# dafyddstephenson/ucla-roms

Hardware: AMD Instinct MI355X
Metric: grid-cell-updates/sec (higher is better)
Workload: dtype f64; 1 GPU; C3: basin 1024x1024x100, NONLIN+SPLIT EOS, T+S, LMD KPP/BKPP/RIMIX/NONLOCAL, dt=300s, ndtfast=60 (nfast=82); NT=2, nfast=82, parallelism=domain decomposition 1x1, halo_transport=none (single rank), fast_exchange_interval=1, exchange_order=none (single rank), s2d_window=True, comm_bootstrap=none (single rank)

## Files before the change

include/roms_gpu.h:

```cpp
#ifndef ROMS_GPU_H
#define ROMS_GPU_H

#ifdef __cplusplus
extern "C" {
#endif

#define ROMS_GPU_ABI_VERSION 23
#define ROMS_MAX_FAST 288

typedef struct roms_dims {
  int Lm, Mm, N, NT;
  int LLm, MMm;
  int np_xi, np_eta, inode, jnode;
  int iSW_corn, jSW_corn;
  int ew_periodic, ns_periodic;
  int west_exchng, east_exchng, south_exchng, north_exchng;
} roms_dims;

#define ROMS_LMD_MIXING   1
#define ROMS_LMD_KPP      2
#define ROMS_LMD_BKPP     4
#define ROMS_LMD_RIMIX    8
#define ROMS_LMD_CONVEC   16
#define ROMS_LMD_NONLOCAL 32
#define ROMS_LMD_ALL      63
#define ROMS_LMD_ICELAND  47
#define ROMS_LMD_DDMIX    64

typedef struct roms_cfg {
  int nonlin_eos;
  int salinity;
  int lmd_mixing;
  int uv_vis2, ts_dif2;
  double dt;
  int ndtfast, nfast;
  double weight[2][ROMS_MAX_FAST];
  double g, rho0, rdrg, rdrg2, Zob, gamma2;
  double Akv_bak, Akt_bak[2];
  double Tcoef, T0, Scoef, S0;
  double theta_s, theta_b, hc;
  int obc;
  double ubind;
  int curvgrid;
  int uv_adv, uv_cor;
  int pot_tides;
  int bulk_frc;
  int adv_isoneutral;
} roms_cfg;

typedef struct roms_tlev {
  int iic, ntstart, forw_start, iif, nfast, kstp, knew, nstp, nrhs, nnew;
} roms_tlev;

enum roms_field {
  ROMS_ALL = -1,
  ROMS_h = 0, ROMS_hinv, ROMS_f, ROMS_fomn, ROMS_pm, ROMS_pn, ROMS_dm_r, ROMS_dn_r, ROMS_dm_u, ROMS_dn_u,
  ROMS_dm_v, ROMS_dn_v, ROMS_dm_p, ROMS_dn_p, ROMS_pmon_u, ROMS_pnom_v, ROMS_rmask, ROMS_pmask, ROMS_umask,
  ROMS_vmask,
  ROMS_Cs_w, ROMS_Cs_r,
  ROMS_zeta, ROMS_ubar, ROMS_vbar, ROMS_u, ROMS_v, ROMS_t, ROMS_FlxU, ROMS_FlxV, ROMS_We, ROMS_Wi,
// ... 37 lines not shown
int roms_gpu_pre_step3d(const roms_tlev *t);
int roms_gpu_set_huv1(const roms_tlev *t);
int roms_gpu_step3d_uv1(const roms_tlev *t);
int roms_gpu_visc3d(const roms_tlev *t);
int roms_gpu_step2d(const roms_tlev *t);
int roms_gpu_step3d_uv2(const roms_tlev *t);
int roms_gpu_step3d_t(const roms_tlev *t);
int roms_gpu_t3dmix(const roms_tlev *t);
int roms_gpu_swr_frac(const roms_tlev *t);
int roms_gpu_set_pipe_frc(int npip, const int *pipe_idx, const double *pipe_flx, const double *pipe_prf,
                          const double *pipe_trc);
int roms_gpu_set_river_frc(int nriv, const double *riv_uflx, const double *riv_vflx, const double *riv_vol,
                           const double *riv_trc);
int roms_gpu_bulk_flux(const roms_tlev *t);
int roms_gpu_set_ub_tune(const double *ub_west, const double *ub_east, const double *ub_south, const double *ub_north);
int roms_gpu_set_depth(const roms_tlev *t);

int roms_gpu_step(roms_tlev *t);
int roms_gpu_init_sequence(roms_tlev *t);

enum roms_case_id { ROMS_CASE_FILAMENT = 0, ROMS_CASE_BASIN = 1, ROMS_CASE_PIPES = 2, ROMS_CASE_RIVERS = 3 };
typedef struct roms_case {
  int case_id, LLm, MMm, N, NT;
  int salinity, nonlin_eos, lmd_mixing;
  double dt; int ndtfast;
  double sizex, sizey;
  int surf_flux;
  int obc;
  double v_sponge;
  int island;
  int curvgrid;
  int uv_adv, uv_cor;
  int bulk_frc;
  int adv_isoneutral;
} roms_case;
int roms_gpu_init_case(const roms_case *c, int device, roms_tlev *t);
int roms_gpu_init_case_comm(const roms_case *c, int np_xi, int np_eta, void *comm, int device, roms_tlev *t);

int roms_gpu_comm_unique_id(void *id128);
int roms_gpu_comm_create(const void *id128, int nranks, int rank, int device, void **comm);
int roms_gpu_comm_create_local(int group, int nranks, int rank, void **comm);
typedef int (*roms_host_allgather_fn)(void *ctx, const void *send, long nbytes, void *recv);
int roms_gpu_comm_create_host(int nranks, int rank, int device, roms_host_allgather_fn allgather, void *ctx,
                              void **comm);
int roms_gpu_comm_destroy(void *comm);
int roms_gpu_halo_transport(void);
int roms_gpu_halo_exchanges(long *per_step, int *fast_interval);
int roms_gpu_halo_overlap(void);
int roms_gpu_s2d_window(void);
#define ROMS_COLPATH_SEG 1
#define ROMS_COLPATH_GLOBAL 2
int roms_gpu_column_path(void);
int roms_gpu_kpp_lean(void);
int roms_gpu_vgrid(void);
int roms_gpu_vgrid2(void);
int roms_gpu_vgrid_check(long out[3]);
int roms_gpu_tracer_pair(long launches[2]);
int roms_gpu_tracer_hstg(long launches[3]);
int roms_gpu_horizontal_path(int out[8]);
int roms_gpu_selftest_zero_fill(long n, int chunks, long *bad);
int roms_gpu_halo_plan(int Lm, int Mm, int np_xi, int np_eta, int inode, int jnode, int ew_periodic,
                       int ns_periodic, int peer[8], long count[8], int strip[4]);
long roms_gpu_halo_map(int Lm, int Mm, int np_xi, int np_eta, int inode, int jnode, int ew_periodic,
                       int ns_periodic, int dir, int unpack, int *i, int *j, long cap);
long roms_gpu_halo_map_wide(int Lm, int Mm, int np_xi, int np_eta, int inode, int jnode, int ew_periodic,
                            int ns_periodic, int width, int dir, int unpack, int *i, int *j, long cap);

#define ROMS_FRC_SURFACE 1
#define ROMS_FRC_BRY     2
int roms_gpu_frc_record(int field_id, int slot, double rec_time, const double *data);
int roms_gpu_frc_interp(double modtime, int kinds);
int roms_gpu_frc_clock(double start_time, int on);
int roms_gpu_set_tide_data(int ntides, const double *ftide, const double *pot_re, const double *pot_im,
                           const double *ztide_re, const double *ztide_im, const double *utide_re,
                           const double *utide_im, const double *vtide_re, const double *vtide_im);
int roms_gpu_set_tides(double time);

#define ROMS_WRT_Z    1
#define ROMS_WRT_UB   2
#define ROMS_WRT_VB   4
#define ROMS_WRT_U    8
#define ROMS_WRT_V    16
#define ROMS_WRT_T    32
#define ROMS_WRT_R    64
#define ROMS_WRT_O    128
#define ROMS_WRT_AKV  256
#define ROMS_WRT_AKT  512
#define ROMS_WRT_AKS  1024
#define ROMS_WRT_HBLS 2048
#define ROMS_WRT_HBBL 4096
#define ROMS_WRT_DEFAULT 63
int roms_gpu_wrt_rst(const char *path, int rec, int total_rec, double time, const roms_tlev *t);
int roms_gpu_wrt_his(const char *path, int rec, int total_rec, double time, const roms_tlev *t, int wrt_mask);
int roms_gpu_io_wait(void);
int roms_gpu_io_tracer_name(int itrc, const char *name, const char *units, const char *long_name);
int roms_gpu_get_init(const char *path, int req_rec, int tindx, roms_tlev *t, double *start_time);

int roms_gpu_diag(const roms_tlev *t, double norms[4]);
int roms_gpu_set_weights(int ndtfast, double weight[2][ROMS_MAX_FAST]);
int roms_gpu_time_steps(roms_tlev *t, int n, double *ms);
enum roms_routine {
  ROMS_R_RHO_EOS = 0, ROMS_R_SET_HUV, ROMS_R_OMEGA, ROMS_R_PRSGRD, ROMS_R_PRE_STEP3D, ROMS_R_SET_HUV1,
  ROMS_R_STEP3D_UV1, ROMS_R_VISC3D, ROMS_R_STEP2D, ROMS_R_STEP3D_UV2, ROMS_R_STEP3D_T, ROMS_R_T3DMIX,
  ROMS_R_LMD_VMIX,
  ROMS_R_K_S2D_FB,
  ROMS_R_K_PRE_UV_SEG,
// ... 15 lines not shown
```

ucla-roms_amd/csrc/k_lmd.hip:

```cpp
#include <cmath>
#include <type_traits>

#include "k_common.h"

namespace roms {
namespace {

constexpr double kRicr = 0.15, kEpssfc = 0.1, kC_Ek = 258.;
constexpr double kZeta_m = -0.2, kA_m = 1.257, kC_m = 8.360, kZeta_s = -1.0, kA_s = -28.86, kC_s = 98.96;
constexpr double kEPS = 1.E-20;
constexpr double kRi0 = 0.7, kNu0m = 1.e-2, kNu0s = 1.e-2, kNuwm = 1.0e-4, kNuws = 0.1e-4, kNu0c = 0.1, kLturb = 10.;
constexpr double kPi = 3.14159265358979323;

__device__ __forceinline__ void ddmix(double t0, double t1, double s0, double s1, double zwk, double& kt,
                                      double& ks) {
  const double A0 = +0.665157E-01, A1 = +0.170907E-01, A2 = -0.203814E-03, A3 = +0.298357E-05,
               A4 = -0.255019E-07, B0 = +0.378110E-02, B1 = -0.846960E-04, C0 = -0.678662E-05,
               D0 = +0.380374E-04, D1 = -0.933746E-06, D2 = +0.791325E-08, E0 = -0.164759E-06,
               F0 = -0.251520E-11, G0 = +0.512857E-12, H0 = -0.302285E-13, Smean = 35.0;
  const double lmd_nu = 1.5e-6, lmd_Rrho0 = 1.9, lmd_nuf = 10.0e-4, lmd_fdd = 0.7, lmd_tdd1 = 0.909,
               lmd_tdd2 = 4.6, lmd_tdd3 = 0.54, lmd_sdd1 = 0.15, lmd_sdd2 = 1.85, lmd_sdd3 = 0.85, eps = 1.E-14;
  const double Tt = 0.5 * (t0 + t1);
  const double Ts = 0.5 * (s0 + s1) - Smean;
  const double Tp = -zwk;
// ... 97 lines not shown
  for (int dj = 0; dj < 2; dj++)
#pragma unroll
    for (int di = 0; di < 3; di++) FE1[dj][di] = (w[dj + 1][di] - w[dj][di]) * m.vm[dj][di];
  const double FEj = FE1[0][1] + cff * (FX[1][1] + FX[0][0] - FX[1][0] - FX[0][1]);
  const double FEjp = FE1[1][1] + cff * (FX[2][1] + FX[1][0] - FX[2][0] - FX[1][1]);
  const double FXi = FX[1][0] + cff * (FE1[1][1] + FE1[0][0] - FE1[0][1] - FE1[1][0]);
  const double FXip = FX[1][1] + cff * (FE1[1][2] + FE1[0][1] - FE1[0][2] - FE1[1][1]);
  return w[1][1] + cff1 * (FXip - FXi + FEjp - FEj);
}

__device__ __forceinline__ void load3x3(const Bounds& b, const EdgeClamp& ec, const double* a, int i, int j,
                                        double (&w)[3][3]) {
#pragma unroll
  for (int dj = 0; dj < 3; dj++)
#pragma unroll
    for (int di = 0; di < 3; di++) w[dj][di] = a[ec.at(b, i - 1 + di, j - 1 + dj)];
}

__global__ void __launch_bounds__(256) k_swr_frac(Dev d, Range R) {
  ROMS_IJ_OR_RETURN(R)
  const Bounds& b = d.b;
  const long ij = IJ(b, i, j), n2 = b.n2;
  const int N = b.N;
  const double mu1 = 0.35, mu2 = 23.0, r1 = 0.58;
  const double attn1 = -1. / mu1, attn2 = -1. / mu2;
  double swdk1 = r1, swdk2 = 1. - swdk1;
  double* __restrict__ sw = d.f.swr_frac + ij;
  const double* __restrict__ Hz = d.f.Hz + ij;
  sw[(long)N * n2] = 1.;
  for (int k = N; k >= 1; k--) {
    const double hz = Hz[(long)(k - 1) * n2];
    const double xi1 = attn1 * hz;
    if (xi1 > -20.) swdk1 = swdk1 * exp(xi1);
    else swdk1 = 0.;
    const double xi2 = attn2 * hz;
    if (xi2 > -20.) swdk2 = swdk2 * exp(xi2);
    else swdk2 = 0.;
    sw[(long)(k - 1) * n2] = swdk1 + swdk2;
  }
}

#ifndef ROMS_KBLS_G
#define ROMS_KBLS_G 16
#endif
constexpr int kKblsG = ROMS_KBLS_G;
#ifndef ROMS_KPP_PFD
#define ROMS_KPP_PFD 1
#endif
constexpr int kKppPfd = ROMS_KPP_PFD;

#ifndef ROMS_KPP_EXT_WAVES
#define ROMS_KPP_EXT_WAVES 3
#endif
template <class C, bool KEEP = false, bool VG = false>
__global__ void __launch_bounds__(64, ROMS_KPP_EXT_WAVES) k_kpp_ext(Dev d, Range E, int tind, int nstp, KppConst kc) {
  ROMS_IJC_OR_RETURN(E)
  const Bounds& b = d.b;
  const Fields& F = d.f;
  const Params& P = d.p;
  const int N = b.N;
  const long n2 = b.n2, ij = IJ(b, i, j), sj = b.nx2;
  const double g = P.g, vonKar = P.vonKar, Ri_inv = 1. / kRicr;
  const C FCc = ColMake<C>::at(d, 0, 0, ij);
  const BufF64 FCg(d.f.colscr);
  constexpr bool kGlb = std::is_same<C, ColGlb>::value;
  static_assert(!KEEP || std::is_same<C, ColLds>::value, "KEEP: the LDS slot");
  const int keep = KEEP ? (P.kpp_fckeep < N ? P.kpp_fckeep : N) : N;
  auto fc_set = [&](int k, double v) {
    if constexpr (kGlb) FCg.st(v, (unsigned)ij * 8u, (unsigned)k * (unsigned)n2 * 8u);
    else if (!KEEP || k <= keep) FCc[k] = v;
  };
  auto fc_get = [&](int k) {
    if constexpr (kGlb) return FCg.ld((unsigned)ij * 8u, (unsigned)k * (unsigned)n2 * 8u);
    else return FCc[k];
  };
  double alpha, beta;
  const double Tt = F.t[ij + (long)(N - 1) * n2 + (long)(nstp - 1) * b.n3];
  if (P.nonlin_eos) {
    const double r01 = 6.793952E-2, r02 = -9.095290E-3, r03 = +1.001685E-4, r04 = -1.120083E-6,
                 r05 = +6.536332E-9, r10 = +0.824493, r11 = -4.08990E-3, r12 = +7.64380E-5,
                 r13 = -8.24670E-7, r14 = +5.38750E-9, rS0 = -5.72466E-3, rS1 = +1.02270E-4,
                 rS2 = -1.65460E-6, r20 = +4.8314E-4;
    const double cff = 1. / P.rho0;
    if (P.salinity) {
      const double Ts = F.t[ij + (long)(N - 1) * n2 + (long)(nstp - 1) * b.n3 + 3 * b.n3], sqrtTs = sqrt(dmax(0., Ts));
      alpha = -cff * (r01 + Tt * (2. * r02 + Tt * (3. * r03 + Tt * (4. * r04 + Tt * 5. * r05))) +
                      Ts * (r11 + Tt * (2. * r12 + Tt * (3. * r13 + Tt * 4. * r14)) + sqrtTs * (rS1 + Tt * 2. * rS2)));
      beta = cff * (r10 + Tt * (r11 + Tt * (r12 + Tt * (r13 + Tt * r14))) + 1.5 * (rS0 + Tt * (rS1 + Tt * rS2)) * sqrtTs +
                    2. * r20 * Ts);
    } else {
      alpha = -cff * (r01 + Tt * (2. * r02 + Tt * (3. * r03 + Tt * (4. * r04 + Tt * 5. * r05))));
      beta = 0.;
    }
  } else {
    alpha = fabs(P.Tcoef);
    beta = P.salinity ? fabs(P.Scoef) : 0.;
  }
  const double sr = F.srflx[ij];
  const double Bo = P.salinity ? g * (alpha * (F.stflx[ij] - sr) - beta * F.stflx[ij + n2]) : g * (alpha * (F.stflx[ij] - sr));
  const double Bosol = g * alpha * sr;
  double ustar;
  if (P.bulk_frc) {
    const double sr_ = F.sustr_r[ij], sv_ = F.svstr_r[ij];
    ustar = sqrt(sqrt(sr_ * sr_ + sv_ * sv_));
  } else {
    const double su0 = F.sustr[ij], su1 = F.sustr[ij + 1], sv0 = F.svstr[ij], sv1 = F.svstr[ij + sj];
    ustar = sqrt(sqrt(0.333333333333 * (su0 * su0 + su1 * su1 + su0 * su1 + sv0 * sv0 + sv1 * sv1 + sv0 * sv1)));
  }
  const double hbl0 = F.hbls[ij], bbl0 = F.hbbl[ij];
  const double rm = F.rmask[ij], ff = F.f[ij];
  F.lmd_Bo[ij] = Bo;
  F.lmd_Bosol[ij] = Bosol;
  F.lmd_ustar[ij] = ustar;

  const unsigned vo = (unsigned)ij * 8u, vx = vo + 8u, vy = vo + (unsigned)sj * 8u, lv = (unsigned)n2 * 8u;
  const BufF64 U(F.u + (long)(tind - 1) * b.n3), V(F.v + (long)(tind - 1) * b.n3), Hz(F.Hz), zr(F.z_r), zw(F.z_w),
      bvf(F.bvf), sw(F.swr_frac), rig(F.lmd_rig);
  VGrid vg{};
  if constexpr (VG) vg = vg_column(d, ij);
  const double zwN = VG ? vg.zw1(N) : zw.ld(vo, (unsigned)N * lv), zw0 = VG ? vg.zw0() : zw.ld(vo, 0);
  double zwc = VG ? vg_zw(vg, N - 1) : 0.;
  const double eh = kEpssfc * hbl0, eb = kEpssfc * bbl0;
  const double eh2 = eh * eh, eb2 = eb * eb;

  auto vtsq = [&](double zrk, double swk, double swm, double bm) {
    const double swdk_r = sqrt(swk * swm);
    const double zscale = zwN - zrk;
    const double Bfsfc = Bo + Bosol * (1. - swdk_r);
    const double ws = wscale_ws(zscale, Bfsfc, hbl0, ustar, rm, vonKar);
    return 1.8 * kc.Vtc * ws * sqrt(dmax(1.e-5, bm));
  };
  struct Lv { double u0, u1, v0, v1, hz, zr, zw, swm, bm; };
  auto ldlev = [&](int k, Lv& L, bool need_sw) {
    const unsigned o = (unsigned)(k - 1) * lv, ow = (unsigned)k * lv;
    L.u0 = U.ld(vo, o); L.u1 = U.ld(vx, o); L.v0 = V.ld(vo, o); L.v1 = V.ld(vy, o);
    if constexpr (!VG) { L.hz = Hz.ld(vo, o); L.zr = zr.ld(vo, o); L.zw = zw.ld(vo, ow); }
    L.swm = sw.ld(need_sw ? vo : kBufOff, o); L.bm = bvf.ld(vo, o);
  };
  auto fc_term = [&](double u0p, double u1p, double v0p, double v1p, double hzp, double u0, double u1, double v0,
                     double v1, double hz, double zwk, double bk) {
    const double cu = zwN - zwk, cd = zwk - zw0;
    const double cff_up = cu * cu, cff_dn = cd * cd;
    const double Kern = cff_up * cff_dn / ((cff_up + eh2) * (cff_dn + eb2));
    const double du = u0p + u1p - u0 - u1;
    const double dv = v0p + v1p - v0 - v1;
    const double hh = hz + hzp;
    return Kern * (0.5 * (du * du + dv * dv) / hh - 0.5 * hh * (Ri_inv * bk + kC_Ek * ff * ff));
  };
  const unsigned oN = (unsigned)(N - 1) * lv;
  double u0p = U.ld(vo, oN), u1p = U.ld(vx, oN);
  double v0p = V.ld(vo, oN), v1p = V.ld(vy, oN);
  double hzp = VG ? zwN - zwc : Hz.ld(vo, oN), zrp = VG ? vg.zr(N) : zr.ld(vo, oN);
  double swc = sw.ld(vo, oN), bc = bvf.ld(vo, oN);
  Lv cur{};
  if (N - 1 >= 1) ldlev(N - 1, cur, true);
  double FCk = 0.;
  fc_set(N, 0.);
  double Crp = FCk + vtsq(zrp, sw.ld(vo, (unsigned)N * lv), swc, bc);
  int kbls = Crp < 0. ? N : 0;
  double cr_k = Crp, cr_kp = 0., zr_k = zrp, zr_kp = 0.;
  const bool skipv = (P.kpp_lean & 1) != 0;
  bool vdone = skipv && __all(kbls != 0);
  for (int k = N - 1; k >= 1; k--) {
    Lv nxt = cur;
    if (k > 1) ldlev(k - 1, nxt, !vdone);
    const unsigned ow = (unsigned)k * lv;
    const double u0 = cur.u0, u1 = cur.u1, v0 = cur.v0, v1 = cur.v1;
    double hz, zrk, zwk;
    if constexpr (VG) {
      const double lo = vg_zw(vg, k - 1);
      zwk = zwc; zrk = vg.zr(k); hz = zwc - lo;
      zwc = lo;
    } else {
      hz = cur.hz; zrk = cur.zr; zwk = cur.zw;
    }
    const double bk = bc;
    if (P.lmd_rimix) {
      const double cff = 0.5 / (zrp - zrk);
      const double dudz = cff * (u0p - u0 + u1p - u1);
      const double dvdz = cff * (v0p - v0 + v1p - v1);
      rig.st(bk / (kRi0 * dmax(dudz * dudz + dvdz * dvdz, 1.E-10)), vo, ow);
    }
    FCk = FCk + fc_term(u0p, u1p, v0p, v1p, hzp, u0, u1, v0, v1, hz, zwk, bk);
    fc_set(k, FCk);
    if (!vdone) {
      const double Cr = FCk + vtsq(zrk, swc, cur.swm, cur.bm);
      if (kbls == 0 && Cr < 0.) {
        kbls = k;
        cr_k = Cr; cr_kp = Crp; zr_k = zrk; zr_kp = zrp;
      }
      Crp = Cr;
      swc = cur.swm;
      vdone = skipv && __all(kbls != 0);
    }
    u0p = u0; u1p = u1; v0p = v0; v1p = v1; hzp = hz; zrp = zrk;
    bc = cur.bm;
    cur = nxt;
  }
  double fc0;
  {
    const double hz1 = hzp;
    const double z_bl = zw0 + 0.25 * hz1;
    const double cu = zwN - z_bl, cd = z_bl - zw0;
    const double cff_up = cu * cu, cff_dn = cd * cd;
    const double Kern = cff_up * cff_dn / ((cff_up + eh2) * (cff_dn + eb2));
    const double su = u0p + u1p, sv = v0p + v1p;
    fc0 = FCk + Kern * (0.5 * (su * su + sv * sv) / hz1 - 0.5 * hz1 * (Ri_inv * bvf.ld(vo, lv) + kC_Ek * ff * ff));
    fc_set(0, fc0);
  }
  double hbl;
  if (kbls > 0) {
    if (kbls == N) hbl = zwN - (VG ? vg.zr(N) : zr.ld(vo, oN));
    else hbl = zwN - (zr_k * cr_kp - zr_kp * cr_k) / (cr_kp - cr_k);
  } else {
    hbl = zwN - zw0;
  }
  F.lmd_hbl[ij] = hbl * rm;
  const double FC0 = fc0;
  double bbl = zwN - zw0;
  int kb = 0;
  double crk = 0., crmk = 0.;
  {
    constexpr int G = kKblsG;
    double crm = 0.;
    for (int k0 = 1; k0 <= keep; k0 += G) {
      double c[G];
#pragma unroll
      for (int q = 0; q < G; q++) c[q] = fc_get(k0 + q <= keep ? k0 + q : keep);
#pragma unroll
      for (int q = 0; q < G; q++) {
        if (kb == 0 && k0 + q <= keep) {
          const double cr = c[q] - FC0;
          if (cr > 0.) { kb = k0 + q; crk = cr; crmk = crm; }
          crm = cr;
        }
      }
      if (__all(kb != 0)) break;
    }
  }
  if constexpr (KEEP) {
    if (keep < N && !__all(kb != 0)) {
      double zwf = VG ? vg_zw(vg, N - 1) : 0.;
      double u0p = U.ld(vo, oN), u1p = U.ld(vx, oN), v0p = V.ld(vo, oN), v1p = V.ld(vy, oN),
             hzp = VG ? zwN - zwf : Hz.ld(vo, oN);
      double FCf = 0.;
      double crp = 0. - FC0;
      int kf = 0;
      double crkf = 0., crmf = 0.;
      for (int k = N - 1; k > keep; k--) {
        const unsigned o = (unsigned)(k - 1) * lv, ow = (unsigned)k * lv;
// ... 238 lines not shown
      rcomp(cur, rvn, rtn, rsn, zk1);
      nv = rvn; nt = rtn; ns = rsn;
    } else {
      rvN = rv; rtN = rt; rsN = rs;
      nv = rv + akv; nt = rt + akt; ns = rs + aks;
    }
    sv = 0.5 * rv + 0.25 * sv + 0.25 * nv + akv;
    st = 0.5 * rt + 0.25 * st + 0.25 * nt + akt;
    ss = 0.5 * rs + 0.25 * ss + 0.25 * ns + aks;
    finish(k, sv, st, ss, zk);
    rv = rvn; rt = rtn; rs = rsn; zk = zk1;
  }
  finish(N, rvN + akv, rtN + akt, rsN + aks, zwN);
  if (!act) return;
  F.hbls[ij] = hbl;
  F.hbbl[ij] = bbl;
  const bool W = !b.ew_periodic && b.west_edge && i == b.istr, E = !b.ew_periodic && b.east_edge && i == b.iend;
  const bool S = !b.ns_periodic && b.south_edge && j == b.jstr, Nn = !b.ns_periodic && b.north_edge && j == b.jend;
  if (W) { F.hbls[ij - 1] = hbl; F.hbbl[ij - 1] = bbl; }
  if (E) { F.hbls[ij + 1] = hbl; F.hbbl[ij + 1] = bbl; }
  if (S) { F.hbls[ij - sj] = hbl; F.hbbl[ij - sj] = bbl; }
  if (Nn) { F.hbls[ij + sj] = hbl; F.hbbl[ij + sj] = bbl; }
  if (W && S) { F.hbls[ij - 1 - sj] = hbl; F.hbbl[ij - 1 - sj] = bbl; }
  if (W && Nn) { F.hbls[ij - 1 + sj] = hbl; F.hbbl[ij - 1 + sj] = bbl; }
  if (E && S) { F.hbls[ij + 1 - sj] = hbl; F.hbbl[ij + 1 - sj] = bbl; }
  if (E && Nn) { F.hbls[ij + 1 + sj] = hbl; F.hbbl[ij + 1 + sj] = bbl; }
}

}

void launch_swr_frac(const Dev& d, hipStream_t s) {
  const Bounds& b = d.b;
  const Range R{b.istr, b.iend, b.jstr, b.jend};
  hipLaunchKernelGGL(k_swr_frac, grid_of(R), dim3(kBX, kBY), 0, s, d, R);
  ExchList L{};
  L.p[0] = d.f.swr_frac; L.nlev[0] = b.N + 1; L.n = 1;
  launch_exchange_list(d, s, L);
}

void launch_lmd_vmix(const Dev& d, hipStream_t s, const Tlev& t, int tind) {
  const Bounds& b = d.b;
  Range E;
  E.i0 = (b.ew_periodic || !b.west_edge) ? b.istr - 1 : b.istr;
  E.i1 = (b.ew_periodic || !b.east_edge) ? b.iend + 1 : b.iend;
  E.j0 = (b.ns_periodic || !b.south_edge) ? b.jstr - 1 : b.jstr;
  E.j1 = (b.ns_periodic || !b.north_edge) ? b.jend + 1 : b.jend;
  const Range R{b.istr, b.iend, b.jstr, b.jend};
  const double vonKar = d.p.vonKar, Cstar = 10., c_s = kC_s, epssfc = kEpssfc, Cv = 1.8, betaT = -0.2;
  KppConst kc;
  kc.Cg = Cstar * vonKar * std::pow(c_s * vonKar * epssfc, 1. / 3.);
  kc.Vtc = Cv * std::sqrt(-betaT / (c_s * epssfc)) / (kRicr * (vonKar * vonKar));
  const int first = t.iic == t.forw_start;
  const bool vge = (d.p.vg & kVgKppExt) != 0, vgi = (d.p.vg & kVgKppInt) != 0;
#define KPP_EXT(C, KEEP, lds)                                                                                       \
  do {                                                                                                              \
    if (vge) hipLaunchKernelGGL((k_kpp_ext<C, KEEP, true>), gridc_of(E), dim3(kCX), lds, s, d, E, tind, t.nstp, kc); \
    else hipLaunchKernelGGL((k_kpp_ext<C, KEEP, false>), gridc_of(E), dim3(kCX), lds, s, d, E, tind, t.nstp, kc);   \
  } while (0)
  if (d.p.kpp_lean & 2)
    KPP_EXT(ColLds, true, col_lds_bytes(1, d.p.kpp_fckeep < b.N ? d.p.kpp_fckeep : b.N));
  else if (d.f.colscr)
    KPP_EXT(ColGlb, false, 0);
  else
    KPP_EXT(ColLds, false, col_lds_bytes(1, b.N));
#undef KPP_EXT
#define KPP_INT(DD, TY, MW, grid, block)                                                                              \
  do {                                                                                                                \
    if (vgi) hipLaunchKernelGGL((k_kpp_int<DD, TY, MW, true>), grid, block, 0, s, d, R, ec, tind, t.nstp, first, kc);  \
    else hipLaunchKernelGGL((k_kpp_int<DD, TY, MW, false>), grid, block, 0, s, d, R, ec, tind, t.nstp, first, kc);     \
  } while (0)
  const EdgeClamp ec = edge_clamp(b);
  if (d.p.kpp_ty && d.p.lmd_rimix) {
    const int ty = d.p.lmd_ddmix ? 4 : (d.p.kpp_ty == 8 || d.p.kpp_ty == 2) ? d.p.kpp_ty : 4;
    dim3 g = gridc_of(R);
    g.y = (g.y + ty - 1) / ty;
    if (d.p.lmd_ddmix) KPP_INT(true, 4, 1, g, dim3(kCX, 4));
    else if (d.p.kpp_ty == 2) KPP_INT(false, 2, 1, g, dim3(kCX, 2));
    else if (d.p.kpp_ty == 8) KPP_INT(false, 8, 1, g, dim3(kCX, 8));
    else if (d.p.kpp_ty == 43)
      hipLaunchKernelGGL((k_kpp_int<false, 4, 3, false>), g, dim3(kCX, 4), 0, s, d, R, ec, tind, t.nstp, first, kc);
    else KPP_INT(false, 4, 1, g, dim3(kCX, 4));
  } else if (d.p.lmd_ddmix) {
    KPP_INT(true, 0, 1, gridc_of(R), dim3(kCX));
  } else {
    KPP_INT(false, 0, 1, gridc_of(R), dim3(kCX));
  }
#undef KPP_INT
  ExchList L{};
  L.p[0] = d.f.Akv; L.nlev[0] = b.N + 1;
  L.p[1] = d.f.hbls; L.nlev[1] = 1;
  L.p[2] = d.f.hbbl; L.nlev[2] = 1;
  L.p[3] = d.f.Akt; L.nlev[3] = (b.N + 1) * b.nTS;
  L.n = 4;
  launch_exchange_list(d, s, L);
}

}
```

ucla-roms_amd/csrc/roms_dev.h:

```cpp
#pragma once
#include <hip/hip_runtime.h>
#include <cstddef>
#include <cstdint>

namespace roms {

constexpr int kMaxFast = 288;
constexpr int kRowAlign = 16;
constexpr int kAlignOff = 14;

struct Bounds {
  int Lm, Mm, N, NT, nTS, nx2;
  long n2, n3, n3w;
  int gx;
  int istr, iend, jstr, jend;
  int istrU, istrR, iendR, jstrV, jstrR, jendR;
  int istrE, iendE, jstrE, jendE;
  int west_edge, east_edge, south_edge, north_edge;
  int ew_periodic, ns_periodic;
  int west_exch, east_exch, south_exch, north_exch;
};

struct Params {
  int nonlin_eos, salinity, lmd, uv_vis2, ts_dif2;
  int lmd_rimix, lmd_convec, lmd_nonlocal;
  int lmd_ddmix;
  int iso;
  int uv_adv, uv_cor;
  int tides;
  int bulk_frc;
  int : 32;
  int s2d_split;
  int colseg;
  int colreg;
  int uv2_fused;
  int chain;
  int seg_order;
  int seg_xg;
  int s2d_fold;
  int hoist;
  int chain_dirz;
  int prs_fuse_uv;
  int : 32;
  int prs_buf;
  int prs_strip;
  int t_strip;
  int visc_stg;
  int t3dmix_stg;
  int kpp_ty;
  int uv1_lds;
  int omega_seg;
  int omega_cw;
  int p_in_rho;
  int omega_hb;
  int preuv_lds;
  int seg_jrows;
  int seg_buf;
  int vgrid2;
  int t_pair;
  int t_hstg;
  int reserved_[5];
  int s2d_k;
  int uv2e_nc, uv2e_nf;
  int npip;
  int nriv, nrivf;
  int curvgrid;
  int obc;
  short kpp_lean;
  short kpp_fckeep;
  short vgrid;
  short vg;
  double ubind;
  double dt, dtfast, g, rho0, vonKar, qp2, gamma2, hc;
  double rdrg, Zob, Tcoef, T0, Scoef, S0;
  double Akv_bak, Akt_bak[2];
};
static_assert(offsetof(Params, s2d_k) == 196 && offsetof(Params, ubind) == 240 && sizeof(Params) == 384,
              "Params: no member from s2d_k on may move");

struct Fields {
  double *h, *hinv, *f, *fomn, *pm, *pn, *dm_r, *dn_r, *dm_u, *dn_u, *dm_v, *dn_v, *dm_p, *dn_p,
      *pmon_u, *pnom_v, *rmask, *pmask, *umask, *vmask;
  double *dndx, *dmde;
  double* ptide;
  double *uwnd, *vwnd, *tair, *qair, *prate, *swrad, *lwrad, *sustr_r, *svstr_r;
  double *Cs_w, *Cs_r;
  double* z_sd;
  double *zeta, *ubar, *vbar, *u, *v, *t;
  double *FlxU, *FlxV, *We, *Wi, *Hz, *Hz_u, *Hz_v, *z_r, *z_w;
  double *rufrc, *rvfrc, *rhoA, *rhoS, *r_D, *Zt_avg1, *DU_avg1, *DV_avg1, *DU_avg2, *DV_avg2,
      *DU_avg_bak, *DV_avg_bak;
  double *rho, *rho1, *qp1, *bvf, *Akv, *Akt, *visc2_r, *visc2_p, *diff2;
  double *hbls, *hbbl, *ghat, *swr_frac;
  double *sustr, *svstr, *stflx, *srflx, *swflx;
  double *ru, *rv, *P, *rhos;
  double *c0, *c1, *c2, *c3;
  double *s0, *s1, *s2, *s3, *s4, *s5, *s6, *s7, *s8, *s9;
  double *lmd_rig, *lmd_hbl, *lmd_bbl, *lmd_Bo, *lmd_Bosol, *lmd_ustar;
  int* pipe_idx;
  double *pipe_flx, *pipe_prf, *pipe_trc;
  double *riv_uflx, *riv_vflx, *riv_vol, *riv_trc;
  int* riv_face;
  int *uv2e_couple, *uv2e_flux;
  double *bzeta[4], *bubar[4], *bvbar[4], *bu[4], *bv[4], *bt[4];
  double* ub[4];
  double* colscr;
  double *dRdx, *dRde, *idRz, *diff3u, *diff3v, *Akz;
  double *iso_dTdz, *iso_FSC, *iso_dTdx, *iso_dTde, *iso_LapT;
};

enum S2dWinField : int {
  kW_zeta, kW_ubar, kW_vbar, kW_h, kW_dn_u, kW_dm_v, kW_pm, kW_pn, kW_swflx, kW_rmask, kW_rhoS, kW_rhoA, kW_umask,
  kW_vmask, kW_rufrc, kW_rvfrc, kW_DU_avg1, kW_DV_avg1, kW_DU_avg2, kW_DV_avg2, kW_Zt_avg1, kW_DU_avg_bak,
  kW_DV_avg_bak, kW_s0, kW_s1, kWinN
// ... 198 lines not shown
  }
  run(Range{R.i0, R.i0 + 1, R.j0, R.j1});
  run(Range{R.i1 - 1, R.i1, R.j0, R.j1});
  run(Range{R.i0 + 2, R.i1 - 2, R.j0, R.j0 + 1});
  run(Range{R.i0 + 2, R.i1 - 2, R.j1 - 1, R.j1});
  edges();
  rim_fork(d, s, L);
  run(Range{R.i0 + 2, R.i1 - 2, R.j0 + 2, R.j1 - 2});
  rim_join(d, s);
}
bool tracer_exch_list(const Dev& d, int tlev, ExchList& L);
void launch_exchange_tracers(const Dev& d, hipStream_t s, int tlev);
bool setup_column_kernels(int N);
void setup_uv1_seg();
void setup_pre_uv_seg();
inline size_t col_smem_bytes(const Dev& d, int nslots) {
  return d.f.colscr ? 0 : (size_t)nslots * (d.b.N + 1) * 64 * sizeof(double);
}
void launch_set_depth(const Dev& d, hipStream_t s, const Tlev& t, bool exchange = true, bool last = false);
void launch_set_huv(const Dev& d, hipStream_t s, const Tlev& t, bool store_huv = true);
void launch_vgrid_check(const Dev& d, hipStream_t s, unsigned long long* cnt);
void launch_set_huv1(const Dev& d, hipStream_t s, const Tlev& t);
bool launch_omega(const Dev& d, hipStream_t s, const Tlev& t, double hcff = 0.0);
void setup_omega_seg();
bool omega_takes_seg(const Dev& d, int width);
int s2d_edge_mode(const Dev& d);
int s2d_edge_modes_taken(bool reset = false);
long t_pair_launches(int bit, long add = 0, bool reset = false);
long t_hstg_launches(int bit, long add = 0, bool reset = false);
bool prsgrd_takes_strips(const Dev& d, bool with_uv, int& jA, int& jB, int& nstrip);
double pre_step3d_dtau(const Dev& d, const Tlev& t);
void launch_rho_eos(const Dev& d, hipStream_t s, const Tlev& t, int tidx);
void launch_prsgrd(const Dev& d, hipStream_t s, const Tlev& t, int uv_up = -1, bool p_ready = false);
bool launch_tracer_strip(const Dev& d, hipStream_t s, const Range& R, int mode, bool up, bool hb_done, int nnew,
                         int nrhs, double dtau, double cf_stp, double cf_bak, int nstp, int& jA, int& jB);
bool p_in_rho(const Dev& d);
bool prsgrd_can_fuse_uv(const Dev& d);
void launch_pre_step3d(const Dev& d, hipStream_t s, const Tlev& t, bool uv_done = false, bool hb_done = false);
void launch_step3d_uv1(const Dev& d, hipStream_t s, const Tlev& t, bool uv_done = false);
void launch_visc3d(const Dev& d, hipStream_t s, const Tlev& t);
void launch_step2d(const Dev& d, hipStream_t s, const Tlev& t, const double* w1, const double* w2);
void launch_step3d_uv2(const Dev& d, hipStream_t s, const Tlev& t);
void launch_step3d_t(const Dev& d, hipStream_t s, const Tlev& t, bool exchange = true);
void launch_t3dmix(const Dev& d, hipStream_t s, const Tlev& t);
void launch_u3dbc(const Dev& d, hipStream_t s, const Tlev& t);
void launch_river_s2d(const Dev& d, hipStream_t s, int knew);
void launch_bulk_flux(const Dev& d, hipStream_t s, int nrhs);
void launch_river_uv(const Dev& d, hipStream_t s, int nnew, int pred);
void launch_v3dbc(const Dev& d, hipStream_t s, const Tlev& t);
void launch_t3dbc(const Dev& d, hipStream_t s, const Tlev& t, int itrc);
void launch_diag(const Dev& d, hipStream_t s, const Tlev& t, double* out);
void launch_swr_frac(const Dev& d, hipStream_t s);
constexpr int kKppFcKeepMax = 16;
void launch_lmd_vmix(const Dev& d, hipStream_t s, const Tlev& t, int tind);
void launch_iso_slopes(const Dev& d, hipStream_t s);
void launch_iso_diff3(const Dev& d, hipStream_t s, const Tlev& t, int iu0, int iu1, int iv0, int iv1, int j0, int j1);
void launch_iso_exch_diff3(const Dev& d, hipStream_t s);
void launch_iso_tracer(const Dev& d, hipStream_t s, const Tlev& t, int itrc);

}
```

ucla-roms_amd/csrc/roms_shim.cpp:

```cpp
#include <hip/hip_runtime.h>

#include <algorithm>
#include <cmath>
#include <cstdlib>
#include <cstdio>
#include <cstring>
#include <map>
#include <string>
#include <vector>

#include "../../include/roms_gpu.h"
#include "halo.h"
#include "host_init.h"
#include "roms_dev.h"
#include "shim_state.h"

using namespace roms;

namespace {

struct FieldDesc {
  double* d = nullptr;
  long count = 0;
  long hcount = 0;
// ... 647 lines not shown
    }
  }
  P.nonlin_eos = cfg->nonlin_eos; P.salinity = cfg->salinity; P.lmd = cfg->lmd_mixing != 0;
  P.lmd_rimix = (cfg->lmd_mixing & ROMS_LMD_RIMIX) != 0;
  P.lmd_convec = (cfg->lmd_mixing & ROMS_LMD_CONVEC) != 0;
  P.lmd_nonlocal = (cfg->lmd_mixing & ROMS_LMD_NONLOCAL) != 0;
  P.lmd_ddmix = (cfg->lmd_mixing & ROMS_LMD_DDMIX) != 0;
  P.uv_adv = cfg->uv_adv != 0; P.uv_cor = cfg->uv_cor != 0;
  P.tides = cfg->pot_tides != 0;
  P.bulk_frc = cfg->bulk_frc != 0;
  P.iso = cfg->adv_isoneutral != 0;
  P.uv_vis2 = cfg->uv_vis2; P.ts_dif2 = cfg->ts_dif2;
  P.s2d_split = env_on("ROMS_GPU_S2D_SPLIT");
  P.dt = cfg->dt; P.dtfast = cfg->dt / (double)cfg->ndtfast; P.g = cfg->g; P.rho0 = cfg->rho0;
  P.vonKar = 0.41; P.qp2 = 0.0000172; P.gamma2 = cfg->gamma2; P.hc = cfg->hc;
  P.rdrg = cfg->rdrg; P.Zob = cfg->Zob; P.Tcoef = cfg->Tcoef; P.T0 = cfg->T0; P.Scoef = cfg->Scoef; P.S0 = cfg->S0;
  P.Akv_bak = cfg->Akv_bak; P.Akt_bak[0] = cfg->Akt_bak[0]; P.Akt_bak[1] = cfg->Akt_bak[1];
  P.npip = 0;
  if (cfg->obc < 0 || cfg->obc > 15) { g.err = "roms_gpu_init: obc must be a 4-bit edge mask"; return -1; }
  P.obc = cfg->obc & ((dims->ew_periodic ? 0 : 3) | (dims->ns_periodic ? 0 : 12));
  P.ubind = cfg->ubind;
  P.curvgrid = cfg->curvgrid && cfg->uv_adv;
  if (P.obc) P.s2d_split = 1;
  for (int i = 0; i < kMaxFast; i++) { g.w1[i] = cfg->weight[0][i]; g.w2[i] = cfg->weight[1][i]; }
  const bool seg_fits = dims->N <= kSegRows * kSegMaxS && seg_rows_ok(dims->N);
  P.colseg = (size_t)2 * (dims->N + 1) * kCX * sizeof(double) > 64 * 1024 && seg_fits;
  if (env_off("ROMS_GPU_COLSEG")) P.colseg = 0;
  if (env_on("ROMS_GPU_COLSEG")) P.colseg = seg_fits;
  P.colreg = env_int("ROMS_GPU_COLREG", 2, 0, 3);
  P.uv2_fused = !env_off("ROMS_GPU_UV2_FUSED");
  P.chain = !env_off("ROMS_GPU_CHAIN");
  P.seg_order = env_int("ROMS_GPU_SEG_ORDER", 3, 0, 3);
  P.seg_xg = env_int("ROMS_GPU_SEG_XG", 8, 1, 1 << 30);
  P.s2d_fold = !env_on("ROMS_GPU_S2D_EDGES");
  P.chain_dirz = !env_off("ROMS_GPU_CHAIN_DIRZ");
  P.prs_fuse_uv = !env_off("ROMS_GPU_PRS_UV");
  P.uv1_lds = !env_off("ROMS_GPU_UV1_LDS");
  P.p_in_rho = !env_off("ROMS_GPU_P_IN_RHO");
  P.omega_hb = !env_off("ROMS_GPU_OMEGA_HB");
  P.omega_seg = !env_off("ROMS_GPU_OMEGA_SEG");
  {
    const int v = env_int("ROMS_GPU_OMEGA_CW", dims->N > 63 ? 16 : 64, 0, 1 << 30);
    P.omega_cw = v == 32 || v == 64 ? v : 16;
  }
  P.preuv_lds = !env_off("ROMS_GPU_PREUV_LDS");
  P.visc_stg = !env_off("ROMS_GPU_VISC_STG");
  P.t3dmix_stg = !env_off("ROMS_GPU_T3DMIX_STG");
  {
    const int v = env_int("ROMS_GPU_KPP_TY", 4, 0, 43);
    P.kpp_ty = v == 0 || v == 2 || v == 8 || v == 43 ? v : 4;
  }
  P.kpp_lean = (short)env_int("ROMS_GPU_KPP_LEAN", 7, 0, 7);
  P.kpp_fckeep = (short)env_int("ROMS_GPU_KPP_FCKEEP", kKppFcKeepMax, 1, kKppFcKeepMax);
  P.vgrid = (short)env_int("ROMS_GPU_VGRID", kVgDefault, 0, kVgAll);
  P.vgrid2 = env_int("ROMS_GPU_VGRID2", kVg2Default, 0, kVg2All);
  P.vg = 0;
  g.vgrid_valid = false;
  g.t_pair_cfg = env_int("ROMS_GPU_T_PAIR", kTPairDefault, 0, kTPairAll);
  P.t_pair = 0;
  g.akt_same = false;
  (void)t_pair_launches(0, 0, true);
  g.t_hstg_cfg = env_int("ROMS_GPU_T_HSTG", P.colseg ? kTHstgDefault : kTHstgDefaultCol, 0, kTHstgAll);
  P.t_hstg = g.t_hstg_cfg & ~kTHstgHz;
  (void)t_hstg_launches(0, 0, true);
  P.hoist = !env_off("ROMS_GPU_HOIST");
  P.prs_buf = !env_off("ROMS_GPU_PRS_BUF");
  P.prs_strip = !env_off("ROMS_GPU_PRS_STRIP");
  P.t_strip = env_on("ROMS_GPU_T_STRIP");
  P.seg_buf = !env_off("ROMS_GPU_SEG_BUF");
  P.seg_jrows = env_int("ROMS_GPU_SEG_JROWS", kSegJMax < 2 ? kSegJMax : 2, 1, kSegJMax);
  bool col_global = (size_t)2 * (dims->N + 1) * kCX * sizeof(double) > 64 * 1024;
  if (env_on("ROMS_GPU_COL_GLOBAL")) col_global = true;
  if (env_off("ROMS_GPU_COL_GLOBAL")) col_global = false;
  setup_uv1_seg();
  setup_pre_uv_seg();
  setup_omega_seg();
  if (!col_global && !setup_column_kernels(dims->N)) {
    g.err = "roms_gpu_init: N too large for the LDS column kernels (2*(N+1)*512 B > 160 KB)";
    return -2;
  }
  CHECK_HIP(hipStreamCreateWithFlags(&g.s, hipStreamNonBlocking));
  g.guard = env_on("ROMS_GPU_GUARD");
  const Bounds& b = g.d.b;
  auto field = [&](int id) -> int {
    const long n = field_count(id, b);
    double* p = nullptr;
    CHECK_HIP(dev_alloc(p, n));
    g.f[id].d = p;
    g.f[id].count = n;
    g.f[id].hcount = field_count(id, g.hb);
    g.f[id].planar = planar_field(id);
    *field_slot(g.d.f, id) = p;
    return 0;
  };
  auto planar2d = [&](int id) { return planar_field(id) && field_count(id, b) <= 4 * b.n2; };
  {
    long n = 11 * dev_alloc_size(b.n2);
    for (int id = 0; id < ROMS_NFIELDS; id++)
      if (planar2d(id)) n += dev_alloc_size(field_count(id, b));
    if (n * 8 < 2147483648L - (1L << 20)) {
      CHECK_HIP(hipMalloc(&g.arena, (size_t)n * sizeof(double)));
      g.arena_n = n;
      g.arena_used = 0;
    }
  }
  for (int id = 0; id < ROMS_NFIELDS; id++)
// ... 191 lines not shown

int roms_gpu_s2d_window(void) {
  REQUIRE_INIT_NOJOIN();
  return g.d.w2.base ? 1 : 0;
}

int roms_gpu_column_path(void) {
  REQUIRE_INIT_NOJOIN();
  return (g.d.p.colseg ? ROMS_COLPATH_SEG : 0) | (g.d.f.colscr ? ROMS_COLPATH_GLOBAL : 0);
}

int roms_gpu_vgrid(void) {
  REQUIRE_INIT_NOJOIN();
  return g.d.p.vgrid + (g.vgrid_valid ? 256 : 0);
}

int roms_gpu_vgrid2(void) {
  REQUIRE_INIT_NOJOIN();
  return g.d.p.vgrid2 + (g.vgrid_valid ? 256 : 0);
}

int roms_gpu_tracer_pair(long launches[2]) {
  REQUIRE_INIT_NOJOIN();
  if (launches) { launches[0] = t_pair_launches(kTPairPre); launches[1] = t_pair_launches(kTPairCor); }
  return g.t_pair_cfg + (g.akt_same ? 256 : 0);
}

int roms_gpu_tracer_hstg(long launches[3]) {
  REQUIRE_INIT_NOJOIN();
  if (launches) {
    launches[0] = t_hstg_launches(kTHstgPre);
    launches[1] = t_hstg_launches(kTHstgCor);
    launches[2] = t_hstg_launches(kTHstgHz);
  }
  return g.t_hstg_cfg + (g.vgrid_valid ? 256 : 0);
}

int roms_gpu_vgrid_check(long out[3]) {
  REQUIRE_INIT_RO();
  if (!out) { g.err = "roms_gpu_vgrid_check: null argument"; return -1; }
  unsigned long long* cnt = (unsigned long long*)shim_scratch_small(3);
  if (!cnt) { g.err = "roms_gpu_vgrid_check: out of device memory"; return -2; }
  CHECK_HIP(hipMemsetAsync(cnt, 0, 3 * sizeof(unsigned long long), g.s));
  launch_vgrid_check(g.d, g.s, cnt);
  unsigned long long h[3] = {0, 0, 0};
  CHECK_HIP(copy_on(h, cnt, sizeof(h), hipMemcpyDeviceToHost, g.s));
  for (int q = 0; q < 3; q++) out[q] = (long)h[q];
  return post_launch();
}

int roms_gpu_kpp_lean(void) {
  REQUIRE_INIT_NOJOIN();
  return g.d.p.kpp_lean + 256 * g.d.p.kpp_fckeep;
}

int roms_gpu_horizontal_path(int out[8]) {
  REQUIRE_INIT_NOJOIN();
  if (!out) { g.err = "roms_gpu_horizontal_path: null argument"; return -1; }
  const Dev& d = g.d;
  int jA = 0, jB = -1, nstrip = 0;
  const bool strips = prsgrd_takes_strips(d, prsgrd_can_fuse_uv(d), jA, jB, nstrip);
  out[0] = s2d_edge_mode(d);
  out[1] = strips ? 1 : 0;
  out[2] = strips ? nstrip : 0;
  out[3] = strips ? jA : 0;
  out[4] = strips ? jB : -1;
  out[5] = omega_takes_seg(d, d.b.iend - d.b.istr + 1) ? 1 : 0;
  out[6] = s2d_edge_modes_taken();
  out[7] = 0;
  return 0;
}

int roms_gpu_halo_exchanges(long* per_step, int* fast_interval) {
  REQUIRE_INIT_NOJOIN();
  if (per_step) *per_step = g.step_exch;
  if (fast_interval) *fast_interval = g.d.p.s2d_k;
  return 0;
}

int roms_gpu_step2d(const roms_tlev* t) {
  REQUIRE_INIT_NOJOIN();
  REQUIRE_HALO_OK();
  const Tlev T = to_tlev(t);
  launch_step2d(g.d, g.s, T, g.w1, g.w2);
  if (T.iif == T.nfast) vg_set(true);
  return post_launch();
}

int roms_gpu_rho_eos(int tidx, const roms_tlev* t) {
  REQUIRE_INIT();
  launch_rho_eos(g.d, g.s, to_tlev(t), tidx);
  return post_launch();
}
int roms_gpu_lmd_vmix(int tind, const roms_tlev* t) {
  REQUIRE_INIT();
  if (!g.cfg.lmd_mixing) { g.err = "roms_gpu_lmd_vmix: library initialised without lmd_mixing"; return -4; }
  if (tind < 1 || tind > 3) { g.err = "roms_gpu_lmd_vmix: bad time index"; return -1; }
  launch_lmd_vmix(g.d, g.s, to_tlev(t), tind);
  akt_lmd_done();
  return post_launch();
}
int roms_gpu_swr_frac(const roms_tlev* t) {
  (void)t;
  REQUIRE_INIT();
  launch_swr_frac(g.d, g.s);
  g.have_swr = true;
// ... 531 lines not shown
```

ucla-roms_amd/romsgpu/__init__.py:

```python
import ctypes
import os

import numpy as np

_HERE = os.path.dirname(os.path.abspath(__file__))
_PKG = os.path.dirname(_HERE)
LIB_PATH = os.environ.get("ROMS_GPU_LIB") or os.path.join(_PKG, "libromsgpu.so")
MAX_FAST = 288

FIELDS = ["h", "hinv", "f", "fomn", "pm", "pn", "dm_r", "dn_r", "dm_u", "dn_u", "dm_v", "dn_v", "dm_p", "dn_p",
          "pmon_u", "pnom_v", "rmask", "pmask", "umask", "vmask", "Cs_w", "Cs_r",
          "zeta", "ubar", "vbar", "u", "v", "t", "FlxU", "FlxV", "We", "Wi", "Hz", "Hz_u", "Hz_v", "z_r", "z_w",
          "rufrc", "rvfrc", "rhoA", "rhoS", "r_D", "Zt_avg1", "DU_avg1", "DV_avg1", "DU_avg2", "DV_avg2",
          "DU_avg_bak", "DV_avg_bak", "rho", "rho1", "qp1", "bvf", "Akv", "Akt", "visc2_r", "visc2_p", "diff2",
          "hbls", "hbbl", "ghat", "swr_frac", "sustr", "svstr", "stflx", "srflx", "swflx", "ru", "rv"] + \
         ["%s_%s" % (v, e) for v in ("zeta", "ubar", "vbar", "u", "v", "t") for e in ("west", "east", "south", "north")] + \
         ["dndx", "dmde", "ptide", "uwnd", "vwnd", "tair", "qair", "prate", "swrad", "lwrad", "sustr_r", "svstr_r"]
FIELD_ID = {n: i for i, n in enumerate(FIELDS)}
CASE_FILAMENT, CASE_BASIN, CASE_PIPES, CASE_RIVERS = 0, 1, 2, 3
LMD_MIXING, LMD_KPP, LMD_BKPP, LMD_RIMIX, LMD_CONVEC, LMD_NONLOCAL = 1, 2, 4, 8, 16, 32
LMD_DDMIX = 64
LMD_ALL = 63
LMD_ICELAND = 47

# ... 406 lines not shown
    def bulk_flux(self):
        self._chk(self.L.roms_gpu_bulk_flux(ctypes.byref(self.t)), "bulk_flux")

    def _r(self, fn):
        self._chk(getattr(self.L, "roms_gpu_" + fn)(ctypes.byref(self.t)), fn)

    def set_HUV(self): self._r("set_huv")
    def omega(self): self._r("omega")
    def prsgrd(self): self._r("prsgrd")
    def pre_step3d(self): self._r("pre_step3d")
    def set_HUV1(self): self._r("set_huv1")
    def step3d_uv1(self): self._r("step3d_uv1")
    def visc3d(self): self._r("visc3d")
    def step2d(self): self._r("step2d")
    def step3d_uv2(self): self._r("step3d_uv2")
    def step3d_t(self): self._r("step3d_t")
    def t3dmix(self): self._r("t3dmix")
    def set_depth(self): self._r("set_depth")
    def swr_frac(self): self._r("swr_frac")
    def init_sequence(self): self._r("init_sequence")

    def step(self, n=1):
        for _ in range(n):
            self._r("step")

    def time_routine(self, routine, nsteps):
        ms = ctypes.c_double()
        n = ctypes.c_long()
        self._chk(self.L.roms_gpu_time_routine(ROUTINES.index(routine), nsteps, ctypes.byref(self.t), ctypes.byref(ms),
                                               ctypes.byref(n)), "time_routine")
        return ms.value, n.value

    def selftest_zero_fill(self, n, chunks=1):
        nz = ctypes.c_long()
        self._chk(self.L.roms_gpu_selftest_zero_fill(ctypes.c_long(n), ctypes.c_int(chunks), ctypes.byref(nz)),
                  "selftest_zero_fill")
        return nz.value

    def halo_transport(self):
        r = self.L.roms_gpu_halo_transport()
        return {1: "ipc", 0: "rccl", -1: "ipc-timeout"}.get(r, "error")

    def halo_overlap(self):
        return bool(self.L.roms_gpu_halo_overlap())

    def s2d_window(self):
        return bool(self.L.roms_gpu_s2d_window())

    def kpp_lean(self):
        r = self.L.roms_gpu_kpp_lean()
        self._chk(min(r, 0), "kpp_lean")
        return r % 256, r // 256

    def vgrid(self):
        r = self.L.roms_gpu_vgrid()
        self._chk(min(r, 0), "vgrid")
        return r % 256, bool(r // 256)

    def vgrid2(self):
        r = self.L.roms_gpu_vgrid2()
        self._chk(min(r, 0), "vgrid2")
        return r % 256, bool(r // 256)

    def tracer_pair(self):
        n = (ctypes.c_long * 2)(0, 0)
        r = self.L.roms_gpu_tracer_pair(n)
        self._chk(min(r, 0), "tracer_pair")
        return r % 256, bool(r // 256), (n[0], n[1])

    def tracer_hstg(self):
        n = (ctypes.c_long * 3)(0, 0, 0)
        r = self.L.roms_gpu_tracer_hstg(n)
        self._chk(min(r, 0), "tracer_hstg")
        return r % 256, bool(r // 256), (n[0], n[1], n[2])

    def vgrid_mismatch(self):
        out = (ctypes.c_long * 3)()
        self._chk(self.L.roms_gpu_vgrid_check(out), "vgrid_check")
        return out[0], out[1], out[2]

    def column_path(self):
        r = self.L.roms_gpu_column_path()
        self._chk(min(r, 0), "column_path")
        return bool(r & 1), bool(r & 2)

    def horizontal_path(self):
        out = (ctypes.c_int * 8)()
        self._chk(self.L.roms_gpu_horizontal_path(out), "horizontal_path")
        return {"edges": out[0], "strips": (out[2], out[3], out[4]) if out[1] else None, "omega_seg": bool(out[5])}

    def fast_step_edge_modes(self):
        out = (ctypes.c_int * 8)()
        self._chk(self.L.roms_gpu_horizontal_path(out), "horizontal_path")
        return {m for m in range(3) if out[6] >> m & 1}

    def halo_exchanges(self):
        n, k = ctypes.c_long(), ctypes.c_int()
        self._chk(self.L.roms_gpu_halo_exchanges(ctypes.byref(n), ctypes.byref(k)), "halo_exchanges")
        return n.value, k.value

    def diag(self):
        out = (ctypes.c_double * 4)()
        self._chk(self.L.roms_gpu_diag(ctypes.byref(self.t), out), "diag")
        return list(out)

    def time(self, dt):
# ... 41 lines not shown
```

Measured before the change: 2.477 billion cell-updates/s.

## Add multi-level register prefetch ring to KPP external column sweep

The KPP surface-layer kernel's downward level loop now keeps a ring buffer of PF+2 levels in registers, loading PF levels ahead instead of one. When the vertical-grid path is active it also prefetches the Cs_w/Cs_r coefficients. Default depth is 3, set through an environment variable. The aim is to hide global-memory latency in the serial column walk, at the cost of more registers, so the occupancy bound drops to 2 waves per SIMD for PF>1.

```diff
diff --git a/include/roms_gpu.h b/include/roms_gpu.h
--- a/include/roms_gpu.h
+++ b/include/roms_gpu.h
@@ -5,7 +5,7 @@
 extern "C" {
 #endif
 
-#define ROMS_GPU_ABI_VERSION 23
+#define ROMS_GPU_ABI_VERSION 24
 #define ROMS_MAX_FAST 288
 
 typedef struct roms_dims {
@@ -149,6 +149,7 @@
 #define ROMS_COLPATH_GLOBAL 2
 int roms_gpu_column_path(void);
 int roms_gpu_kpp_lean(void);
+int roms_gpu_kpp_pf(void);
 int roms_gpu_vgrid(void);
 int roms_gpu_vgrid2(void);
 int roms_gpu_vgrid_check(long out[3]);
diff --git a/ucla-roms_amd/csrc/k_lmd.hip b/ucla-roms_amd/csrc/k_lmd.hip
--- a/ucla-roms_amd/csrc/k_lmd.hip
+++ b/ucla-roms_amd/csrc/k_lmd.hip
@@ -173,8 +173,9 @@
 #ifndef ROMS_KPP_EXT_WAVES
 #define ROMS_KPP_EXT_WAVES 3
 #endif
-template <class C, bool KEEP = false, bool VG = false>
-__global__ void __launch_bounds__(64, ROMS_KPP_EXT_WAVES) k_kpp_ext(Dev d, Range E, int tind, int nstp, KppConst kc) {
+constexpr int kpp_ext_waves(int pf) { return pf <= 1 ? ROMS_KPP_EXT_WAVES : 2; }
+template <class C, bool KEEP = false, bool VG = false, int PF = 1>
+__global__ void __launch_bounds__(64, kpp_ext_waves(PF)) k_kpp_ext(Dev d, Range E, int tind, int nstp, KppConst kc) {
   ROMS_IJC_OR_RETURN(E)
   const Bounds& b = d.b;
   const Fields& F = d.f;
@@ -251,13 +252,19 @@
     const double ws = wscale_ws(zscale, Bfsfc, hbl0, ustar, rm, vonKar);
     return 1.8 * kc.Vtc * ws * sqrt(dmax(1.e-5, bm));
   };
-  struct Lv { double u0, u1, v0, v1, hz, zr, zw, swm, bm; };
+  struct Lv0 { double u0, u1, v0, v1, hz, zr, zw, swm, bm; };
+  struct Lv1 : Lv0 { double cw, cr; };
+  constexpr bool kCs = VG && PF > 1;
+  using Lv = std::conditional_t<kCs, Lv1, Lv0>;
+  const BufF64 CsW(F.Cs_w), CsR(F.Cs_r);
   auto ldlev = [&](int k, Lv& L, bool need_sw) {
     const unsigned o = (unsigned)(k - 1) * lv, ow = (unsigned)k * lv;
     L.u0 = U.ld(vo, o); L.u1 = U.ld(vx, o); L.v0 = V.ld(vo, o); L.v1 = V.ld(vy, o);
     if constexpr (!VG) { L.hz = Hz.ld(vo, o); L.zr = zr.ld(vo, o); L.zw = zw.ld(vo, ow); }
+    if constexpr (kCs) { L.cw = CsW.ld(0u, (unsigned)(k - 1) * 8u); L.cr = CsR.ld(0u, (unsigned)k * 8u); }
     L.swm = sw.ld(need_sw ? vo : kBufOff, o); L.bm = bvf.ld(vo, o);
   };
+  auto ring_level = [](int k) { return __builtin_amdgcn_readfirstlane(k >= 1 ? k : 1); };
   auto fc_term = [&](double u0p, double u1p, double v0p, double v1p, double hzp, double u0, double u1, double v0,
                      double v1, double hz, double zwk, double bk) {
     const double cu = zwN - zwk, cd = zwk - zw0;
@@ -274,7 +281,14 @@
   double hzp = VG ? zwN - zwc : Hz.ld(vo, oN), zrp = VG ? vg.zr(N) : zr.ld(vo, oN);
   double swc = sw.ld(vo, oN), bc = bvf.ld(vo, oN);
   Lv cur{};
-  if (N - 1 >= 1) ldlev(N - 1, cur, true);
+  Lv S[PF + 2] = {};
+  if constexpr (PF == 1) {
+    if (N - 1 >= 1) ldlev(N - 1, cur, true);
+  } else {
+    S[0].u0 = u0p; S[0].u1 = u1p; S[0].v0 = v0p; S[0].v1 = v1p; S[0].swm = swc; S[0].bm = bc;
+#pragma unroll
+    for (int q = 1; q <= PF; q++) ldlev(ring_level(N - q), S[q], true);
+  }
   double FCk = 0.;
   fc_set(N, 0.);
   double Crp = FCk + vtsq(zrp, sw.ld(vo, (unsigned)N * lv), swc, bc);
@@ -282,20 +296,21 @@
   double cr_k = Crp, cr_kp = 0., zr_k = zrp, zr_kp = 0.;
   const bool skipv = (P.kpp_lean & 1) != 0;
   bool vdone = skipv && __all(kbls != 0);
-  for (int k = N - 1; k >= 1; k--) {
-    Lv nxt = cur;
-    if (k > 1) ldlev(k - 1, nxt, !vdone);
+  auto level = [&](int k, const Lv& cur, double u0p, double u1p, double v0p, double v1p, double swk, double bk) {
     const unsigned ow = (unsigned)k * lv;
     const double u0 = cur.u0, u1 = cur.u1, v0 = cur.v0, v1 = cur.v1;
     double hz, zrk, zwk;
-    if constexpr (VG) {
+    if constexpr (kCs) {
+      const double lo = vg.zw(k - 1, cur.cw);
+      zwk = zwc; zrk = vg.zr(k, cur.cr); hz = zwc - lo;
+      zwc = lo;
+    } else if constexpr (VG) {
       const double lo = vg_zw(vg, k - 1);
       zwk = zwc; zrk = vg.zr(k); hz = zwc - lo;
       zwc = lo;
     } else {
       hz = cur.hz; zrk = cur.zr; zwk = cur.zw;
     }
-    const double bk = bc;
     if (P.lmd_rimix) {
       const double cff = 0.5 / (zrp - zrk);
       const double dudz = cff * (u0p - u0 + u1p - u1);
@@ -305,18 +320,42 @@
     FCk = FCk + fc_term(u0p, u1p, v0p, v1p, hzp, u0, u1, v0, v1, hz, zwk, bk);
     fc_set(k, FCk);
     if (!vdone) {
-      const double Cr = FCk + vtsq(zrk, swc, cur.swm, cur.bm);
+      const double Cr = FCk + vtsq(zrk, swk, cur.swm, cur.bm);
       if (kbls == 0 && Cr < 0.) {
         kbls = k;
         cr_k = Cr; cr_kp = Crp; zr_k = zrk; zr_kp = zrp;
       }
       Crp = Cr;
-      swc = cur.swm;
+      if constexpr (PF == 1) swc = cur.swm;
       vdone = skipv && __all(kbls != 0);
     }
-    u0p = u0; u1p = u1; v0p = v0; v1p = v1; hzp = hz; zrp = zrk;
-    bc = cur.bm;
-    cur = nxt;
+    hzp = hz; zrp = zrk;
+  };
+  if constexpr (PF == 1) {
+    for (int k = N - 1; k >= 1; k--) {
+      Lv nxt = cur;
+      if (k > 1) ldlev(k - 1, nxt, !vdone);
+      level(k, cur, u0p, u1p, v0p, v1p, swc, bc);
+      u0p = cur.u0; u1p = cur.u1; v0p = cur.v0; v1p = cur.v1;
+      bc = cur.bm;
+      cur = nxt;
+    }
+  } else {
+    constexpr int M = PF + 2;
+#pragma unroll 1
+    for (int kg = N - 1; kg >= 1; kg -= M) {
+#pragma unroll
+      for (int q = 0; q < M; q++) {
+        const int k = kg - q;
+        if (k >= 1) {
+          const Lv& prv = S[q];
+          const Lv& cur = S[(q + 1) % M];
+          ldlev(ring_level(k - PF), S[(q + M - 1) % M], !vdone);
+          level(k, cur, prv.u0, prv.u1, prv.v0, prv.v1, prv.swm, prv.bm);
+          if (k == 1) { u0p = cur.u0; u1p = cur.u1; v0p = cur.v0; v1p = cur.v1; }
+        }
+      }
+    }
   }
   double fc0;
   {
@@ -661,10 +700,21 @@
   kc.Vtc = Cv * std::sqrt(-betaT / (c_s * epssfc)) / (kRicr * (vonKar * vonKar));
   const int first = t.iic == t.forw_start;
   const bool vge = (d.p.vg & kVgKppExt) != 0, vgi = (d.p.vg & kVgKppInt) != 0;
-#define KPP_EXT(C, KEEP, lds)                                                                                       \
-  do {                                                                                                              \
-    if (vge) hipLaunchKernelGGL((k_kpp_ext<C, KEEP, true>), gridc_of(E), dim3(kCX), lds, s, d, E, tind, t.nstp, kc); \
-    else hipLaunchKernelGGL((k_kpp_ext<C, KEEP, false>), gridc_of(E), dim3(kCX), lds, s, d, E, tind, t.nstp, kc);   \
+#define KPP_EXT_PF(C, KEEP, VGF, PF, lds) \
+  hipLaunchKernelGGL((k_kpp_ext<C, KEEP, VGF, PF>), gridc_of(E), dim3(kCX), lds, s, d, E, tind, t.nstp, kc)
+#define KPP_EXT_VG(C, KEEP, VGF, lds)                     \
+  do {                                                    \
+    switch (d.p.kpp_pf) {           \
+      case 2: KPP_EXT_PF(C, KEEP, VGF, 2, lds); break;    \
+      case 3: KPP_EXT_PF(C, KEEP, VGF, 3, lds); break;    \
+      case 4: KPP_EXT_PF(C, KEEP, VGF, 4, lds); break;    \
+      default: KPP_EXT_PF(C, KEEP, VGF, 1, lds); break;   \
+    }                                                     \
+  } while (0)
+#define KPP_EXT(C, KEEP, lds)                  \
+  do {                                         \
+    if (vge) KPP_EXT_VG(C, KEEP, true, lds);   \
+    else KPP_EXT_VG(C, KEEP, false, lds);      \
   } while (0)
   if (d.p.kpp_lean & 2)
     KPP_EXT(ColLds, true, col_lds_bytes(1, d.p.kpp_fckeep < b.N ? d.p.kpp_fckeep : b.N));
@@ -673,6 +723,8 @@
   else
     KPP_EXT(ColLds, false, col_lds_bytes(1, b.N));
 #undef KPP_EXT
+#undef KPP_EXT_VG
+#undef KPP_EXT_PF
 #define KPP_INT(DD, TY, MW, grid, block)                                                                              \
   do {                                                                                                                \
     if (vgi) hipLaunchKernelGGL((k_kpp_int<DD, TY, MW, true>), grid, block, 0, s, d, R, ec, tind, t.nstp, first, kc);  \
diff --git a/ucla-roms_amd/csrc/roms_dev.h b/ucla-roms_amd/csrc/roms_dev.h
--- a/ucla-roms_amd/csrc/roms_dev.h
+++ b/ucla-roms_amd/csrc/roms_dev.h
@@ -59,7 +59,8 @@
   int vgrid2;
   int t_pair;
   int t_hstg;
-  int reserved_[5];
+  int kpp_pf;
+  int reserved_[4];
   int s2d_k;
   int uv2e_nc, uv2e_nf;
   int npip;
@@ -364,6 +365,8 @@
 void launch_diag(const Dev& d, hipStream_t s, const Tlev& t, double* out);
 void launch_swr_frac(const Dev& d, hipStream_t s);
 constexpr int kKppFcKeepMax = 16;
+constexpr int kKppPfMax = 4;
+constexpr int kKppPfDefault = 3;
 void launch_lmd_vmix(const Dev& d, hipStream_t s, const Tlev& t, int tind);
 void launch_iso_slopes(const Dev& d, hipStream_t s);
 void launch_iso_diff3(const Dev& d, hipStream_t s, const Tlev& t, int iu0, int iu1, int iv0, int iv1, int j0, int j1);
diff --git a/ucla-roms_amd/csrc/roms_shim.cpp b/ucla-roms_amd/csrc/roms_shim.cpp
--- a/ucla-roms_amd/csrc/roms_shim.cpp
+++ b/ucla-roms_amd/csrc/roms_shim.cpp
@@ -723,6 +723,10 @@
   }
   P.kpp_lean = (short)env_int("ROMS_GPU_KPP_LEAN", 7, 0, 7);
   P.kpp_fckeep = (short)env_int("ROMS_GPU_KPP_FCKEEP", kKppFcKeepMax, 1, kKppFcKeepMax);
+  {
+    const int v = env_int("ROMS_GPU_KPP_PF", kKppPfDefault, -(1 << 30), 1 << 30);
+    P.kpp_pf = v >= 1 && v <= kKppPfMax ? v : 1;
+  }
   P.vgrid = (short)env_int("ROMS_GPU_VGRID", kVgDefault, 0, kVgAll);
   P.vgrid2 = env_int("ROMS_GPU_VGRID2", kVg2Default, 0, kVg2All);
   P.vg = 0;
@@ -1020,6 +1024,11 @@
 int roms_gpu_kpp_lean(void) {
   REQUIRE_INIT_NOJOIN();
   return g.d.p.kpp_lean + 256 * g.d.p.kpp_fckeep;
+}
+
+int roms_gpu_kpp_pf(void) {
+  REQUIRE_INIT_NOJOIN();
+  return g.d.p.kpp_pf;
 }
 
 int roms_gpu_horizontal_path(int out[8]) {
diff --git a/ucla-roms_amd/romsgpu/__init__.py b/ucla-roms_amd/romsgpu/__init__.py
--- a/ucla-roms_amd/romsgpu/__init__.py
+++ b/ucla-roms_amd/romsgpu/__init__.py
@@ -482,6 +482,11 @@
         self._chk(min(r, 0), "kpp_lean")
         return r % 256, r // 256
 
+    def kpp_pf(self):
+        r = self.L.roms_gpu_kpp_pf()
+        self._chk(min(r, 0), "kpp_pf")
+        return r
+
     def vgrid(self):
         r = self.L.roms_gpu_vgrid()
         self._chk(min(r, 0), "vgrid")
```

After: 2.506 billion cell-updates/s (median of 6 runs). 1.2% higher.
